# laprade117/interactive-unet

Hardware: AMD Instinct MI355X
Metric: voxels/sec (train step + full-volume predict) on 128^3 chunks (higher is better)
Workload: dtype bf16

## Files before the change

### include/iunet.h

```cpp
#ifndef IUNET_H
#define IUNET_H
#ifdef __cplusplus
extern "C" {
#endif

const char* iunet_last_error(void);
int iunet_abi_version(void);

long long iunet_pack_conv3_elems(int Cout, int Cin, int taps, int mode);
int iunet_pack_conv3(int dtype, const void* w, const void* scale, void* dst, int Cout, int Cin, int taps, int mode,
                     void* stream);
long long iunet_pack_first_conv_elems(int Cout, int Cin, int taps);
int iunet_pack_first_conv(int dtype, const void* w, const void* scale, void* dst, int Cout, int Cin, int taps,
                          void* stream);
int iunet_pack_convT(int dtype, const void* w, void* dst, int Cin, int Cout, int npos, void* stream);

int iunet_pack_desc_bytes(void);
int iunet_pack_batch(const void* descs, int n, int quant_max_cout, void* stream);

int iunet_conv3_fwd(int dtype, int nd, const void* x, long long x_sstride, void* y, long long y_sstride,
                    const void* wpk, const void* bias, void* stats, int N, int D, int H, int W, int Cin, int Cout,
                    int epi, int layout, void* stream);
int iunet_conv3_pick_layout(int nd, int N, int D, int H, int W, int Cin, int Cout);
int iunet_conv3_tile_pairs(int nd, int N, int D, int H, int W, int Cin, int Cout);
// ... 235 lines not shown
int iunet_conv3_dgrad_sample_bnstats(int dtype, int nd, const void* dy, long long dy_sstride, void* dz, long long dz_sstride, const void* wpk,
                                     void* stats, const void* yp, long long yp_sstride, const void* mean, const void* invstd, const void* scale,
                                     const void* shift, int N, int D, int H, int W, int Cin, int Cout, int layout, void* stream);
int iunet_gn_relu_bwd_rows(int dtype, const void* dz, long long dz_ss, const void* y, long long y_ss, void* dy, long long dy_ss,
                           const void* gamma, int groups, const void* scale, const void* shift, const void* mean, const void* invstd,
                           void* dgamma, void* dbeta, void* slab, int rows, void* coef, int C, int N, long long vox, void* stream);
int iunet_gn_relu_pool_bwd(int dtype, int nd, const void* dskip, long long ds_ss, const void* dpool, long long dp_ss, const void* y,
                           long long y_ss, void* dy, long long dy_ss, const void* gamma, int groups, const void* scale, const void* shift,
                           const void* mean, const void* invstd, void* dgamma, void* dbeta, void* slab, void* coef, int C, int N, int Do,
                           int Ho, int Wo, void* stream);
int iunet_bn_relu_pool_bwd(int dtype, int nd, const void* dskip, long long ds_ss, const void* dpool, long long dp_ss,
                           const void* y, long long y_ss, void* dy, long long dy_ss, const void* mean, const void* invstd,
                           const void* gamma, const void* scale, const void* shift, void* dgamma, void* dbeta, void* slab,
                           void* coef, int C, int N, int Do, int Ho, int Wo, void* stream);
int iunet_maxpool_bwd(int dtype, int nd, const void* z, long long z_ss, const void* dpool, long long dp_ss, void* dz,
                      long long dz_ss, int add_skip, int C, int N, int Do, int Ho, int Wo, void* stream);
int iunet_head_loss_num_parts(int N, long long vox);
int iunet_head_loss_fwd(int dtype, const void* x, long long x_ss, int C0, const void* w, const void* bias, int ncls,
                        const void* target, const void* weight, int tdtype, int kind, void* slab, void* out4, void* coef,
                        int N, long long vox, void* stream);
int iunet_head_loss_bwd_num_parts(int N, long long vox, int ncls, int C0);
int iunet_head_loss_bwd(int dtype, const void* x, long long x_ss, int C0, const void* w, const void* bias, int ncls,
                        const void* target, const void* weight, int tdtype, const void* coef, float loss_scale, void* dx,
                        long long dx_ss, void* dwslab, int N, long long vox, void* stream);
int iunet_head_loss_fwd_act(int dtype, const void* x, long long x_ss, int C0, const void* w, const void* bias, int ncls,
                            const void* target, const void* weight, int tdtype, int kind, void* slab, void* out4, void* coef,
                            const void* in_scale, const void* in_shift, int N, long long vox, void* stream);
int iunet_head_loss_bwd_act(int dtype, const void* x, long long x_ss, int C0, const void* w, const void* bias, int ncls,
                            const void* target, const void* weight, int tdtype, const void* coef, float loss_scale, void* dx,
                            long long dx_ss, void* dwslab, const void* in_scale, const void* in_shift, int N, long long vox,
                            void* stream);
int iunet_reduce_slab(void* slab, int nparts, long long n, void* out, float alpha, int accumulate, void* stream);
int iunet_conv3_wgrad_blocks(int nd, int N, int D, int H, int W, int Cin, int Cout);
long long iunet_conv3_wgrad_slab_floats(int nd, int N, int D, int H, int W, int Cin, int Cout);
int iunet_conv3_wgrad(int dtype, int nd, const void* x, long long x_ss, const void* dy, long long dy_ss, void* slab,
                      void* dW, float alpha, int N, int D, int H, int W, int Cin, int Cout, void* stream);
int iunet_conv3_wgrad_act(int dtype, int nd, const void* x, long long x_ss, const void* dy, long long dy_ss, void* slab,
                          void* dW, float alpha, const void* x_scale, const void* x_shift, int N, int D, int H, int W,
                          int Cin, int Cout, void* stream);
int iunet_pack_convT_dgrad(int dtype, const void* w, void* dst, int Cin, int Cout, int npos, void* stream);
int iunet_convT_dgrad(int dtype, int nd, const void* dy, long long dy_ss, void* dx, long long dx_ss, const void* wpk,
                      int N, int D, int H, int W, int Cin, int Cout, void* stream);
int iunet_convT_wgrad_blocks(int nd, int N, int D, int H, int W, int Cin, int Cout);
int iunet_convT_wgrad(int dtype, int nd, const void* x, long long x_ss, const void* dy, long long dy_ss, void* wslab,
                      void* bslab, void* dW, void* db, int N, int D, int H, int W, int Cin, int Cout, void* stream);
int iunet_first_conv_wgrad_blocks(int nd, int N, int D, int H, int W);
int iunet_first_conv_wgrad(int dtype, int nd, const void* x, int in_dtype, const long long* in_strides, const void* dy,
                           long long dy_ss, void* slab, void* dW, int N, int D, int H, int W, int Cin, int Cout,
                           void* stream);
int iunet_first_conv_wgrad_bn(int dtype, int nd, const void* x, int in_dtype, const long long* in_strides, const void* dz,
                              long long dz_ss, const void* y, long long y_ss, const void* mean, const void* invstd,
                              const void* coef, const void* scale, const void* shift, void* slab, void* dW, int N, int D, int H,
                              int W, int Cin, int Cout, void* stream);
int iunet_check_finite(const void* g, long long n, void* flag, void* stream);
int iunet_adamw_step(void* p, const void* g, void* m, void* v, long long n, float lr, float b1, float b2, float eps,
                     float wd, int step, float grad_scale_inv, const void* skip_flag, void* stream);

int iunet_train_state_init(void* state, float loss_scale, int dynamic, void* stream);
int iunet_head_loss_bwd_dev(int dtype, const void* x, long long x_ss, int C0, const void* w, const void* bias, int ncls,
                            const void* target, const void* weight, int tdtype, const void* coef, const void* state, void* dx,
                            long long dx_ss, void* dwslab, const void* in_scale, const void* in_shift, int N, long long vox,
                            void* stream);
int iunet_head_bn_bwd_ok(int C0, int ncls);
int iunet_head_bn_bwd(int dtype, const void* y, long long y_ss, int C0, const void* w, const void* bias, int ncls, const void* target,
                      const void* weight, int tdtype, const void* coef, float loss_scale, const void* state, const void* scale,
                      const void* shift, const void* mean, const void* invstd, const void* gamma, void* dgamma, void* dbeta, void* dy,
                      long long dy_ss, void* dwslab, void* bnslab, void* bncoef, void* dl_scratch, int N, long long vox, void* stream);
int iunet_head_gn_bwd(int dtype, const void* y, long long y_ss, int C0, const void* w, const void* bias, int ncls, const void* target,
                      const void* weight, int tdtype, const void* coef, float loss_scale, const void* state, const void* scale,
                      const void* shift, const void* mean, const void* invstd, const void* gamma, int groups, void* dgamma, void* dbeta, void* dy,
                      long long dy_ss, void* dwslab, void* bnslab, void* bncoef, void* dl_scratch, int N, long long vox, void* stream);
int iunet_head_loss_fwd_act_ps(int dtype, const void* x, long long x_ss, int C0, const void* w, const void* bias, int ncls,
                               const void* target, const void* weight, int tdtype, int kind, void* slab, void* out4, void* coef,
                               const void* in_scale, const void* in_shift, int per_sample, int N, long long vox, void* stream);
int iunet_head_grad_scatter(const void* row, void* dw, void* db, int ncls, int C0, void* stream);
int iunet_adamw_step_dev(void* p, const void* g, void* m, void* v, long long n, float lr, float b1, float b2, float eps, float wd,
                         void* state, int check, float world, void* stream);

typedef struct iunet_train iunet_train;
int iunet_train_create(int dim, int levels, int base, int cin, int ncls, int dtype, int loss_kind, iunet_train** out);
int iunet_train_create_ex(int dim, int levels, int base, int cin, int ncls, int dtype, int loss_kind, int norm, int groups, iunet_train** out);
int iunet_train_create_nested(int dim, int levels, int base, int cin, int ncls, int dtype, int loss_kind, iunet_train** out);
void iunet_train_destroy(iunet_train* t);
long long iunet_train_num_params(const iunet_train* t);
int iunet_train_num_tensors(const iunet_train* t);
int iunet_train_param(const iunet_train* t, int index, char* name, int name_cap, long long* offset, long long* numel);
int iunet_train_num_bn(const iunet_train* t);
long long iunet_train_packed_bytes(const iunet_train* t);
long long iunet_train_workspace_bytes(const iunet_train* t, int N, int D, int H, int W);
int iunet_train_bind(iunet_train* t, void* flat, void* grad, void* m, void* v, void* const* running, void* packed, void* state, void* stream);
int iunet_train_repack(iunet_train* t, void* stream);
int iunet_train_forward_backward(iunet_train* t, const void* x, int in_dtype, const long long* in_strides, const void* target,
                                 const void* weight, int tdtype, int N, int D, int H, int W, void* workspace, void* out4, void* stream);
typedef void (*iunet_train_hook)(void* ctx, int stage);
int iunet_train_forward_backward_hooks(iunet_train* t, const void* x, int in_dtype, const long long* in_strides, const void* target,
                                       const void* weight, int tdtype, int N, int D, int H, int W, void* workspace, void* out4,
                                       iunet_train_hook hook, void* hook_ctx, void* stream);
int iunet_train_update(iunet_train* t, float lr, float b1, float b2, float eps, float wd, float world, void* stream);
int iunet_train_step(iunet_train* t, const void* x, int in_dtype, const long long* in_strides, const void* target, const void* weight,
                     int tdtype, int N, int D, int H, int W, void* workspace, float lr, float b1, float b2, float eps, float wd, void* out4,
                     void* stream);

long long iunet_lk_pack_elems(int nd, int kind, int Cout, int Cin);
int iunet_lk_pack(int dtype, int nd, int kind, const void* w, const void* gamma, const void* beta, const void* mean, const void* var,
                  float eps, void* dst, void* bias_out, int Cout, int Cin, void* stream);
int iunet_lk_stats_parts(int nd, int kind, int N, int D, int H, int W, int Cout);
// ... 100 lines not shown
```

### interactive-unet_amd/csrc/train_misc.hip

```cpp
#include "common.h"

namespace {


struct ConvTDgradParams {
  const void* dy; long long dy_ss;
  void* dx; long long dx_ss;
  const void* wpk;
  int N, D, H, W, Cin, Cout;
};

template <typename T, int ND>
__global__ __launch_bounds__(256) void convT_dgrad_kernel(ConvTDgradParams p) {
  using V8 = V8T<T>;
  constexpr int NPOS = ND == 3 ? 8 : 4;
  const int lane = threadIdx.x & 63, wave = threadIdx.x >> 6;
  const int l15 = lane & 15, q = lane >> 4;
  const int xg = (p.W + 15) / 16;
  const long long rows = (long long)p.D * p.H * xg;
  const long long wid = (long long)blockIdx.x * 4 + wave;
  if (wid >= rows * p.N) return;
  const int n = (int)(wid / rows);
  const long long r = wid - n * rows;
  const int xb = (int)(r % xg), y = (int)((r / xg) % p.H), z = (int)(r / ((long long)xg * p.H));
// ... 280 lines not shown
      for (int t = 0; t < 2; ++t)
#pragma unroll
        for (int u = 0; u < 2; ++u)
#pragma unroll
          for (int j = 0; j < 4; ++j) ws[s * 1024 + (t * 16 + 4 * g + j) * 32 + u * 16 + i16] = acc[c][i][t][u][j];
    }
  }
  if (blockIdx.y == 0) {
    __syncthreads();
    float* red = (float*)smem;
#pragma unroll
    for (int j = 0; j < 8; ++j) red[tid * 8 + j] = bacc[j];
    __syncthreads();
    if (tid < 32) {
      const int pl = tid >> 3, j = tid & 7;
      float sum = 0.f;
      for (int k = pl; k < 256; k += 4) sum += red[k * 8 + j];
      p.bslab[(long long)blockIdx.x * p.Cout + cob * 32 + pl * 8 + j] = sum;
    }
  }
}

__global__ __launch_bounds__(256) void convT_wgrad_reduce_kernel(const float* __restrict__ slab, int nb, int Cin, int Cout, int npos,
                                                                 float* __restrict__ dW) {
  __shared__ f32x4 red[16][16];
  const long long per_b4 = (long long)Cin * Cout * npos / 4;
  const int col4 = threadIdx.x & 15, grp = threadIdx.x >> 4;
  const long long j4 = (long long)blockIdx.x * 16 + col4;
  const f32x4* slab4 = (const f32x4*)slab;
  f32x4 s = f32x4{0.f, 0.f, 0.f, 0.f};
  for (int b = grp; b < nb; b += 16) s += slab4[b * per_b4 + j4];
  red[grp][col4] = s;
  __syncthreads();
  if (grp != 0) return;
#pragma unroll
  for (int g = 1; g < 16; ++g) s += red[g][col4];
  const int ncob = Cout / 32;
#pragma unroll
  for (int k = 0; k < 4; ++k) {
    const long long j = j4 * 4 + k;
    const int c = (int)(j & 31), r = (int)((j >> 5) & 31);
    long long t = j >> 10;
    const int pos = (int)(t % npos); t /= npos;
    const int cob = (int)(t % ncob), cib = (int)(t / ncob);
    dW[((long long)(cib * 32 + r) * Cout + cob * 32 + c) * npos + pos] = s[k];
  }
}

struct FirstWgradParams {
  const void* x; long long sN, sC, sD, sH, sW; int in_dtype;
  const void* dy; long long dy_ss;
  const void* yraw; long long y_ss;
  const float* mean; const float* invstd; const float* coef; const float* scale; const float* shift;
  float* slab;
  int N, D, H, W, Cin, Cout;
  int tilesZ, tilesY, tilesX;
};

__device__ __forceinline__ float load_in2(const void* p, long long off, int dt) {
  switch (dt) {
    case 0: return ((const float*)p)[off];
    case 1: return (float)((const f16*)p)[off];
    case 2: return (float)((const unsigned char*)p)[off] / 255.0f;
    default: return (float)((const bf16*)p)[off];
  }
}

template <typename T, int ND, int CIN>
__global__ __launch_bounds__(256, 2) void first_wgrad_kernel(FirstWgradParams p) {
  using V8 = V8T<T>;
  constexpr int TZ = ND == 3 ? 4 : 1, TY = ND == 3 ? 8 : 16, TX = ND == 3 ? 16 : 32, PADZ = ND == 3 ? 1 : 0;
  constexpr int PZ = TZ + 2 * PADZ, PY = TY + 2, PX = TX + 2, NPIX = PZ * PY * PX, NVOX = TZ * TY * TX;
  constexpr int TAPS = ND == 3 ? 27 : 9, KK = TAPS * CIN, NT = (KK + 15) / 16, KKP = NT * 16;
  constexpr int FX = TX / 16, NKS = NVOX / 32;
  constexpr int PLANE_Y = NVOX * 16 + 64;
  constexpr int XS_BYTES = ((CIN * NPIX * 2 + 255) / 256) * 256;
  extern __shared__ __attribute__((aligned(256))) unsigned char smem[];
  T* xs = (T*)smem;
  unsigned char* dys = smem + XS_BYTES;
  __shared__ __attribute__((aligned(16))) float par[7 * 32];
  if (p.yraw != nullptr && threadIdx.x < 7 * 32) {
    const int k = threadIdx.x >> 5, c = blockIdx.y * 32 + (threadIdx.x & 31);
    par[threadIdx.x] = k == 0 ? p.scale[c] : k == 1 ? p.shift[c] : k == 2 ? p.mean[c] : k == 3 ? p.invstd[c] : p.coef[c * 3 + (k - 4)];
  }
  const unsigned lds_y = (unsigned)(size_t)(__attribute__((address_space(3))) unsigned char*)dys;
  const int tid = threadIdx.x, lane = tid & 63;
  const int wave = __builtin_amdgcn_readfirstlane(tid >> 6);
  const int g = lane >> 4, i16 = lane & 15, q = i16 >> 2, pp = i16 & 3, gh = g >> 1, gl = g & 1;
  const int cob = blockIdx.y;
  const unsigned laneY = lds_y + (pp >> 1) * PLANE_Y + (pp & 1) * 8 + (gh * 16 + gl * 8 + q) * 16;
  int col_off[NT];
#pragma unroll
  for (int ct = 0; ct < NT; ++ct) {
    const int kk = ct * 16 + i16, kc = kk < KK ? kk : 0;
    const int tap = kc / CIN, c = kc % CIN;
    const int dz = ND == 3 ? tap / 9 : 0, dy_ = (tap / 3) % 3, dx = tap % 3;
    col_off[ct] = c * NPIX + (dz * PY + dy_) * PX + dx;
  }
  f32x4 acc[2][NT];
#pragma unroll
  for (int t = 0; t < 2; ++t)
#pragma unroll
    for (int ct = 0; ct < NT; ++ct) acc[t][ct] = f32x4{0, 0, 0, 0};
  const int tps = p.tilesZ * p.tilesY * p.tilesX, ntiles = tps * p.N;
  const long long plane = (long long)p.D * p.H * p.W * 8;
  constexpr int XIT = (NPIX * CIN + 255) / 256, YIT = NVOX * 4 / 256;
  float xr[XIT];
  u32x4 yr[YIT], yw[YIT];
  unsigned oky = 0;
  auto load_tile = [&](int tile) {
    oky = 0;
    const int n = tile / tps;
    int trem = tile - n * tps;
    const int tz_i = trem / (p.tilesY * p.tilesX);
    trem -= tz_i * p.tilesY * p.tilesX;
    const int ty_i = trem / p.tilesX, tx_i = trem - ty_i * p.tilesX;
    const int z0 = tz_i * TZ, y0 = ty_i * TY, x0 = tx_i * TX;
#pragma unroll
    for (int k = 0; k < XIT; ++k) {
      const int it = tid + k * 256;
      const int c = it / NPIX, pix = it - c * NPIX;
      const int px = pix % PX, t2 = pix / PX, py = t2 % PY, pz = t2 / PY;
      const int gz = z0 + pz - PADZ, gy = y0 + py - 1, gx = x0 + px - 1;
      float v = 0.f;
      if (it < NPIX * CIN && (unsigned)gz < (unsigned)p.D && (unsigned)gy < (unsigned)p.H && (unsigned)gx < (unsigned)p.W)
        v = load_in2(p.x, n * p.sN + c * p.sC + gz * p.sD + gy * p.sH + gx * p.sW, p.in_dtype);
      xr[k] = v;
    }
    const T* dyin = (const T*)p.dy + (long long)n * p.dy_ss + (long long)cob * 4 * plane;
#pragma unroll
    for (int it = 0; it < YIT; ++it) {
      const int idx = tid + it * 256, pl = idx / NVOX, pix = idx - pl * NVOX;
      const int px = pix % TX, t2 = pix / TX, py = t2 % TY, pz = t2 / TY;
      const int gz = z0 + pz, gy = y0 + py, gx = x0 + px;
      u32x4 v = u32x4{0u, 0u, 0u, 0u};
      if (gz < p.D && gy < p.H && gx < p.W) v = *(const u32x4*)(dyin + pl * plane + (((long long)gz * p.H + gy) * p.W + gx) * 8);
      yr[it] = v;
      oky |= (gz < p.D && gy < p.H && gx < p.W) ? (1u << it) : 0u;
      if (p.yraw != nullptr) {
        u32x4 w = u32x4{0u, 0u, 0u, 0u};
        if (gz < p.D && gy < p.H && gx < p.W)
          w = *(const u32x4*)((const T*)p.yraw + (long long)n * p.y_ss + (long long)(cob * 4 + pl) * plane + (((long long)gz * p.H + gy) * p.W + gx) * 8);
        yw[it] = w;
      }
    }
  };
  auto commit_tile = [&]() {
#pragma unroll
    for (int k = 0; k < XIT; ++k) {
      const int it = tid + k * 256;
      if (it < NPIX * CIN) xs[it] = from_f32<T>(xr[k]);
    }
#pragma unroll
    for (int it = 0; it < YIT; ++it) {
      const int idx = tid + it * 256, pl = idx / NVOX, pix = idx - pl * NVOX;
      u32x4 v = yr[it];
      if (p.yraw != nullptr && ((oky >> it) & 1u)) {
        const V8 g = __builtin_bit_cast(V8, v), yy = __builtin_bit_cast(V8, yw[it]);
        V8 o;
        const f32x4* pp = (const f32x4*)(par + pl * 8);
        float cs[7][8];
#pragma unroll
        for (int k = 0; k < 7; ++k) {
          const f32x4 lo = pp[k * 8], hi = pp[k * 8 + 1];
#pragma unroll
          for (int j = 0; j < 4; ++j) { cs[k][j] = lo[j]; cs[k][4 + j] = hi[j]; }
        }
#pragma unroll
        for (int j = 0; j < 8; ++j) {
          const float yv = to_f32<T>(yy[j]);
          const float zv = to_f32<T>(from_f32<T>(fmaf(cs[0][j], yv, cs[1][j])));
          const float d = zv > 0.f ? to_f32<T>(g[j]) : 0.f;
          const float xh = (yv - cs[2][j]) * cs[3][j];
          o[j] = from_f32<T>(cs[4][j] * (d - cs[5][j] - xh * cs[6][j]));
        }
        v = __builtin_bit_cast(u32x4, o);
      }
      *(u32x4*)(dys + pl * PLANE_Y + pix * 16) = v;
    }
  };
  if ((int)blockIdx.x < ntiles) load_tile(blockIdx.x);
  for (int tile = blockIdx.x; tile < ntiles; tile += gridDim.x) {
    __syncthreads();
    commit_tile();
    __syncthreads();
    if (tile + (int)gridDim.x < ntiles) load_tile(tile + gridDim.x);
    for (int ks = wave; ks < NKS; ks += 4) {
      const int f = 2 * ks + gh;
      const int xh = f % FX, row = f / FX, fy = row % TY, fz = row / TY;
      const int vbase = (fz * PY + fy) * PX + xh * 16 + gl * 8;
      const V8 a0 = tr_frag2<T>(laneY + (unsigned)(2 * ks * 256), 64);
      const V8 a1 = tr_frag2<T>(laneY + (unsigned)(2 * ks * 256) + 2 * PLANE_Y, 64);
#pragma unroll
      for (int ct = 0; ct < NT; ++ct) {
        V8 b;
#pragma unroll
        for (int j = 0; j < 8; ++j) b[j] = xs[vbase + j + col_off[ct]];
        acc[0][ct] = mfma16<T>(a0, b, acc[0][ct]);
        acc[1][ct] = mfma16<T>(a1, b, acc[1][ct]);
      }
    }
  }
  __syncthreads();
  float* red = (float*)smem;
#pragma unroll
  for (int t = 0; t < 2; ++t)
#pragma unroll
    for (int ct = 0; ct < NT; ++ct)
#pragma unroll
      for (int j = 0; j < 4; ++j) red[(wave * 32 + t * 16 + 4 * g + j) * KKP + ct * 16 + i16] = acc[t][ct][j];
  __syncthreads();
  float* slab = p.slab + ((long long)blockIdx.x * p.Cout + cob * 32) * KKP;
  for (int i = tid; i < 32 * KKP; i += 256)
    slab[i] = red[i] + red[32 * KKP + i] + red[2 * 32 * KKP + i] + red[3 * 32 * KKP + i];
}

__global__ __launch_bounds__(256) void first_wgrad_reduce_kernel(const float* __restrict__ slab, int nb, int Cout, int Cin, int taps,
                                                                 int KKP, float* __restrict__ dW) {
  __shared__ float red[8][32];
  const int total = Cout * Cin * taps;
  const int o = threadIdx.x & 31, grp = threadIdx.x >> 5;
  const int i = blockIdx.x * 32 + o;
  float s = 0.f;
  if (i < total) {
    const int tap = i % taps, c = (i / taps) % Cin, co = i / (taps * Cin);
// ... 78 lines not shown

int iunet_convT_wgrad_blocks(int nd, int N, int D, int H, int W, int Cin, int Cout) {
  if (N < 1 || D < 1 || H < 1 || W < 1 || Cin < 32 || Cout < 32) return 0;
  const int TZ = nd == 3 ? 2 : 1, TY = nd == 3 ? 4 : 8, TX = 16;
  const long long ntiles = (long long)N * ((D + TZ - 1) / TZ) * ((H + TY - 1) / TY) * ((W + TX - 1) / TX);
  const int nci = (Cin / 32) % 2 == 0 ? 2 : 1;
  const int pairs = (Cin / 32 / nci) * (Cout / 32);
  long long nb = (512 + pairs - 1) / pairs;
  if (nb > ntiles) nb = ntiles;
  return (int)(nb < 1 ? 1 : nb);
}

int iunet_convT_wgrad(int dtype, int nd, const void* x, long long x_ss, const void* dy, long long dy_ss, void* wslab,
                      void* bslab, void* dW, void* db, int N, int D, int H, int W, int Cin, int Cout, void* stream) {
  DT_OK(dtype);
  IUNET_REQUIRE(x && dy && wslab && bslab && dW && db, "convT_wgrad: null pointer");
  IUNET_REQUIRE(Cin >= 32 && Cout >= 32 && Cin % 32 == 0 && Cout % 32 == 0, "convT_wgrad: channels must be positive multiples of 32");
  IUNET_REQUIRE(nd == 2 || nd == 3, "convT_wgrad: nd must be 2 or 3");
  IUNET_REQUIRE_GRID("convT_wgrad", N, D, H, W);
  ConvTWgradParams p;
  p.x = x; p.x_ss = x_ss; p.dy = dy; p.dy_ss = dy_ss; p.wslab = (float*)wslab; p.bslab = (float*)bslab;
  p.N = N; p.D = D; p.H = H; p.W = W; p.Cin = Cin; p.Cout = Cout;
  const int TZ = nd == 3 ? 2 : 1, TY = nd == 3 ? 4 : 8, TX = 16;
  p.tilesZ = (D + TZ - 1) / TZ; p.tilesY = (H + TY - 1) / TY; p.tilesX = (W + TX - 1) / TX;
  const int nb = iunet_convT_wgrad_blocks(nd, N, D, H, W, Cin, Cout);
  const int npos = nd == 3 ? 8 : 4;
  const int nvi = 128, nvo = nd == 3 ? 1024 : 512;
  const int lds = 4 * (nvi * 16 + 64) + 4 * (nvo * 16 + 64);
  const int nci = (Cin / 32) % 2 == 0 ? 2 : 1;
  dim3 grid(nb, Cin / 32 / nci, Cout / 32);
#define CTW(TT, NDV) do { if (nci == 2) { IUNET_SET_MAX_LDS((convT_wgrad_kernel<TT, NDV, 2>), lds); \
      hipLaunchKernelGGL((convT_wgrad_kernel<TT, NDV, 2>), grid, dim3(256), lds, (hipStream_t)stream, p); } \
    else { IUNET_SET_MAX_LDS((convT_wgrad_kernel<TT, NDV, 1>), lds); \
      hipLaunchKernelGGL((convT_wgrad_kernel<TT, NDV, 1>), grid, dim3(256), lds, (hipStream_t)stream, p); } } while (0)
  if (dtype == 0) { if (nd == 3) CTW(f16, 3); else CTW(f16, 2); } else { if (nd == 3) CTW(bf16, 3); else CTW(bf16, 2); }
#undef CTW
  const long long total = (long long)Cin * Cout * npos;
  hipLaunchKernelGGL(convT_wgrad_reduce_kernel, dim3((unsigned)(total / 64)), dim3(256), 0, (hipStream_t)stream,
                     (const float*)wslab, nb, Cin, Cout, npos, (float*)dW);
  IUNET_CHECK_HIP(hipGetLastError());
  return iunet_reduce_slab(bslab, nb, Cout, db, 1.0f, 0, stream);
}

int iunet_first_conv_wgrad_blocks(int nd, int N, int D, int H, int W) {
  if (N < 1 || D < 1 || H < 1 || W < 1) return 0;
  const int TZ = nd == 3 ? 4 : 1, TY = nd == 3 ? 8 : 16, TX = nd == 3 ? 16 : 32;
  const long long ntiles = (long long)N * ((D + TZ - 1) / TZ) * ((H + TY - 1) / TY) * ((W + TX - 1) / TX);
  return (int)(ntiles < 512 ? ntiles : 512);
}

static int first_wgrad_impl(int dtype, int nd, const void* x, int in_dtype, const long long* in_strides, const void* dy,
                            long long dy_ss, void* slab, void* dW, int N, int D, int H, int W, int Cin, int Cout,
                            const void* yraw, long long y_ss, const float* mean, const float* invstd, const float* coef,
                            const float* scale, const float* shift, void* stream) {
  DT_OK(dtype);
  IUNET_REQUIRE(x && dy && slab && dW && in_strides, "first_conv_wgrad: null pointer");
  IUNET_REQUIRE(Cin >= 1 && Cin <= 4 && Cout >= 32 && Cout % 32 == 0, "first_conv_wgrad: Cin 1..4, Cout a positive multiple of 32");
  IUNET_REQUIRE(nd == 2 || nd == 3, "first_conv_wgrad: nd must be 2 or 3");
  IUNET_REQUIRE(in_dtype >= 0 && in_dtype <= 3, "first_conv_wgrad: bad input dtype %d", in_dtype);
  IUNET_REQUIRE_GRID("first_conv_wgrad", N, D, H, W);
  FirstWgradParams p;
  p.x = x; p.sN = in_strides[0]; p.sC = in_strides[1]; p.sD = in_strides[2]; p.sH = in_strides[3]; p.sW = in_strides[4];
  p.in_dtype = in_dtype; p.dy = dy; p.dy_ss = dy_ss; p.slab = (float*)slab;
  p.yraw = yraw; p.y_ss = y_ss; p.mean = mean; p.invstd = invstd; p.coef = coef; p.scale = scale; p.shift = shift;
  p.N = N; p.D = D; p.H = H; p.W = W; p.Cin = Cin; p.Cout = Cout;
  const int TZ = nd == 3 ? 4 : 1, TY = nd == 3 ? 8 : 16, TX = nd == 3 ? 16 : 32;
  p.tilesZ = (D + TZ - 1) / TZ; p.tilesY = (H + TY - 1) / TY; p.tilesX = (W + TX - 1) / TX;
  const int nb = iunet_first_conv_wgrad_blocks(nd, N, D, H, W);
  const int taps = nd == 3 ? 27 : 9, KKP = ((taps * Cin + 15) / 16) * 16;
  const int npix = (nd == 3 ? 6 : 1) * (TY + 2) * (TX + 2);
  const int xs_bytes = ((Cin * npix * 2 + 255) / 256) * 256;
  int lds = xs_bytes + 4 * (512 * 16 + 64);
  if (lds < 4 * 32 * KKP * 4) lds = 4 * 32 * KKP * 4;
  dim3 grid(nb, Cout / 32);
#define FW(TT, NDV, CI) do { IUNET_SET_MAX_LDS((first_wgrad_kernel<TT, NDV, CI>), lds); \
    hipLaunchKernelGGL((first_wgrad_kernel<TT, NDV, CI>), grid, dim3(256), lds, (hipStream_t)stream, p); } while (0)
#define FW_CIN(TT, NDV) switch (Cin) { case 1: FW(TT, NDV, 1); break; case 2: FW(TT, NDV, 2); break; case 3: FW(TT, NDV, 3); break; default: FW(TT, NDV, 4); break; }
  if (dtype == 0) { if (nd == 3) { FW_CIN(f16, 3) } else { FW_CIN(f16, 2) } }
  else            { if (nd == 3) { FW_CIN(bf16, 3) } else { FW_CIN(bf16, 2) } }
#undef FW_CIN
#undef FW
  const int total = Cout * Cin * taps;
  hipLaunchKernelGGL(first_wgrad_reduce_kernel, dim3((total + 31) / 32), dim3(256), 0, (hipStream_t)stream,
                     (const float*)slab, nb, Cout, Cin, taps, KKP, (float*)dW);
  IUNET_CHECK_HIP(hipGetLastError());
  return IUNET_OK;
}

int iunet_first_conv_wgrad(int dtype, int nd, const void* x, int in_dtype, const long long* in_strides, const void* dy,
                           long long dy_ss, void* slab, void* dW, int N, int D, int H, int W, int Cin, int Cout,
                           void* stream) {
  return first_wgrad_impl(dtype, nd, x, in_dtype, in_strides, dy, dy_ss, slab, dW, N, D, H, W, Cin, Cout, nullptr, 0, nullptr,
                          nullptr, nullptr, nullptr, nullptr, stream);
}

int iunet_first_conv_wgrad_bn(int dtype, int nd, const void* x, int in_dtype, const long long* in_strides, const void* dz,
                              long long dz_ss, const void* y, long long y_ss, const void* mean, const void* invstd,
                              const void* coef, const void* scale, const void* shift, void* slab, void* dW, int N, int D, int H,
                              int W, int Cin, int Cout, void* stream) {
  IUNET_REQUIRE(y && mean && invstd && coef && scale && shift, "first_conv_wgrad_bn: null pointer");
  return first_wgrad_impl(dtype, nd, x, in_dtype, in_strides, dz, dz_ss, slab, dW, N, D, H, W, Cin, Cout, y, y_ss,
                          (const float*)mean, (const float*)invstd, (const float*)coef, (const float*)scale,
                          (const float*)shift, stream);
}

}
```

### interactive-unet_amd/csrc/train_net.hip

```cpp
#include "common.h"
#include "pack_desc.h"
#include <algorithm>
#include <cstdio>
#include <cstdlib>
#include <string>
#include <vector>

namespace {

long long align256(long long v) { return (v + 255) & ~255ll; }
bool env_on(const char* name) { const char* e = getenv(name); return e != nullptr && e[0] != 0; }

struct TParam { std::string name; long long off, numel; };

struct TPack {
  int cout = 0, cin = 0, dg = 0;
  long long buf[2] = {-1, -1};
  long long elems[2] = {0, 0};
};

struct TConv {
  std::string name;
  int ci, co, l, first;
  long long w, gamma, beta;
// ... 545 lines not shown
                             WS + L.dy, (long long)c0 * v0, F(L.hslab), F(L.bnslab), F(L.bncoef), WS + L.dz[kl] ,
                             N, v0, stream);
      dy_ready = kl;
    } else if (n->head_act)
      rc = iunet_head_loss_bwd_dev(dt, WS + L.y[kl], (long long)c0 * v0, c0, P + n->head_w, P + n->head_b, n->ncls, target, weight, tdtype, F(L.coef),
                                   n->state, WS + L.dz[kl], (long long)c0 * v0, F(L.hslab), F(L.scale[kl]), F(L.shift[kl]), N, v0, stream);
    else
      rc = iunet_head_loss_bwd_dev(dt, WS + L.z[kl], (long long)c0 * v0, c0, P + n->head_w, P + n->head_b, n->ncls, target, weight, tdtype, F(L.coef),
                                   n->state, WS + L.dz[kl], (long long)c0 * v0, F(L.hslab), nullptr, nullptr, N, v0, stream);
    if (rc) return rc;
    rc = iunet_reduce_slab(F(L.hslab), nparts, (long long)n->ncls * (c0 + 1), F(L.htmp), 1.0f, 0, stream);
    if (rc) return rc;
    rc = iunet_head_grad_scatter(F(L.htmp), G + n->head_w, G + n->head_b, n->ncls, c0, stream);
    if (rc) return rc;
  }
  auto conv_bwd = [&](int k, const void* dzp, long long dz_ss, const void* xp, long long x_ss, void* dxp, long long dx_ss, int x_act,
                      const void* dpool, long long dpool_ss, int feeds) -> int {
    const TConv& c = n->conv[k];
    int d, h, w;
    dims(c.l, d, h, w);
    const long long v = vox(c.l);
    void* dy = WS + L.dy;
    const void* y = WS + L.y[k];
    if (k == dy_ready) {
    } else if (n->norm == 1 && dpool != nullptr) {
      int dn, hn, wn;
      dims(c.l + 1, dn, hn, wn);
      rc = iunet_gn_relu_pool_bwd(dt, dim, dzp, dz_ss, dpool, dpool_ss, y, c.co * v, dy, c.co * v, P + c.gamma, n->groups, F(L.scale[k]), F(L.shift[k]),
                                  F(L.mean[k]), F(L.invstd[k]), G + c.gamma, G + c.beta, F(L.bnslab), F(L.bncoef), c.co, N, dn, hn, wn, stream);
    } else if (n->norm == 1) {
      const int rows = bw_ready[k] > 0 ? bw_ready[k] : 0;
      bw_ready[k] = -1;
      rc = iunet_gn_relu_bwd_rows(dt, dzp, dz_ss, y, c.co * v, dy, c.co * v, P + c.gamma, n->groups, F(L.scale[k]), F(L.shift[k]), F(L.mean[k]), F(L.invstd[k]),
                                  G + c.gamma, G + c.beta, rows > 0 ? F(L.stats) : F(L.bnslab), rows, F(L.bncoef), c.co, N, v, stream);
    } else if (dpool != nullptr) {
      int dn, hn, wn;
      dims(c.l + 1, dn, hn, wn);
      rc = iunet_bn_relu_pool_bwd(dt, dim, dzp, dz_ss, dpool, dpool_ss, y, c.co * v, dy, c.co * v, F(L.mean[k]), F(L.invstd[k]), P + c.gamma,
                                  F(L.scale[k]), F(L.shift[k]), G + c.gamma, G + c.beta, F(L.bnslab), F(L.bncoef), c.co, N, dn, hn, wn, stream);
    } else if (bw_ready[k] >= 0) {
      const int nparts = bw_ready[k];
      bw_ready[k] = -1;
      rc = iunet_bn_relu_bwd_apply(dt, dzp, dz_ss, y, c.co * v, c.first ? nullptr : dy, c.co * v, F(L.mean[k]), F(L.invstd[k]), P + c.gamma,
                                   F(L.scale[k]), F(L.shift[k]), G + c.gamma, G + c.beta, F(L.stats), nparts, F(L.bncoef), c.co, N, v, stream);
    } else {
      rc = iunet_bn_relu_bwd(dt, dzp, dz_ss, nullptr, dz_ss, y, c.co * v, c.first ? nullptr : dy, c.co * v, F(L.mean[k]), F(L.invstd[k]), P + c.gamma,
                             F(L.scale[k]), F(L.shift[k]), G + c.gamma, G + c.beta, F(L.bnslab), F(L.bncoef), c.co, N, v, stream);
    }
    if (rc) return rc;
    float* gw = G + c.w;
    if (c.first && n->norm == 1)
      return iunet_first_conv_wgrad(dt, dim, x, in_dtype, in_strides, dy, c.co * v, F(L.wslab), gw, N, d, h, w, c.ci, c.co, stream);
    if (c.first)
      return iunet_first_conv_wgrad_bn(dt, dim, x, in_dtype, in_strides, dzp, dz_ss, y, c.co * v, F(L.mean[k]), F(L.invstd[k]), F(L.bncoef),
                                       F(L.scale[k]), F(L.shift[k]), F(L.wslab), gw, N, d, h, w, c.ci, c.co, stream);
    if (x_act < 0) rc = iunet_conv3_wgrad(dt, dim, xp, x_ss, dy, c.co * v, F(L.wslab), gw, 1.0f, N, d, h, w, c.ci, c.co, stream);
    else rc = iunet_conv3_wgrad_act(dt, dim, xp, x_ss, dy, c.co * v, F(L.wslab), gw, 1.0f, F(L.scale[x_act]), F(L.shift[x_act]), N, d, h, w, c.ci,
                                    c.co, stream);
    if (rc) return rc;
    long long woff;
    int fused = 0;
    const int lay = pack_pick(c.dgr, dim, N, d, h, w, false, feeds >= 0 && (n->fuse_bw || n->gn_bw), &woff, &fused);
    if (lay < 0) return lay;
    if (fused && n->fuse_bw) {
      rc = iunet_conv3_dgrad_bnstats_lay(dt, dim, dy, c.co * v, dxp, dx_ss, K + woff, F(L.stats), WS + L.y[feeds], c.ci * v, F(L.mean[feeds]),
                                         F(L.invstd[feeds]), F(L.scale[feeds]), F(L.shift[feeds]), N, d, h, w, c.co, c.ci, lay, stream);
      bw_ready[feeds] = iunet_conv3_stats_parts(dim, N, d, h, w, c.ci, 2);
    } else {
      int gn_rows = 0;
      if (n->norm == 1 && fused && n->gn_bw)
        gn_rows = iunet_conv3_sample_stats_rows(dt, dim, N, d, h, w, c.co, c.ci, lay);
      if (gn_rows > 0) {
        rc = iunet_conv3_dgrad_sample_bnstats(dt, dim, dy, c.co * v, dxp, dx_ss, K + woff, F(L.stats), WS + L.y[feeds], c.ci * v, F(L.mean[feeds]),
                                              F(L.invstd[feeds]), F(L.scale[feeds]), F(L.shift[feeds]), N, d, h, w, c.co, c.ci, lay, stream);
        bw_ready[feeds] = gn_rows;
      } else {
        rc = iunet_conv3_fwd(dt, dim, dy, c.co * v, dxp, dx_ss, K + woff, nullptr, nullptr, N, d, h, w, c.co, c.ci, 0, lay, stream);
      }
    }
    return rc;
  };
  if (n->nested) {
    auto node_conv2_bwd = [&](int s, int i, int m, const void* dpool, long long dpool_ss) -> int {
      const long long v = vox(i);
      const int c = n->ch[i], k1 = 2 * s, k2 = k1 + 1;
      const bool fused = conv2_fused(i);
      const void* x2 = fused ? (const void*)(WS + L.y[k1]) : (const void*)(WS + L.z[k1]);
      const void* dzp = nullptr;
      long long dz_ss = 0;
      if (k2 != dy_ready) {
        const void* sp[8];
        long long ss[8];
        int K_ = 0;
        for (int jj = m + 1; jj < lv - i; ++jj) {
          const int q = n->node_at[i * lv + jj];
          sp[K_] = WS + L.ndcat[q] + (long long)m * c * v * 2; ss[K_++] = (long long)(jj + 1) * c * v;
        }
        if (i >= 1) { sp[K_] = WS + L.dT[n->node_at[(i - 1) * lv + m + 1]]; ss[K_++] = (long long)c * v; }
        if (K_ + (dpool != nullptr) == 1) {
          dzp = sp[0]; dz_ss = ss[0];
        } else {
          const TConv& cc = n->conv[k2];
          int d, h, w;
          dims(i, d, h, w);
          rc = iunet_bn_relu_sum_bwd(dt, dim, K_, sp, ss, dpool, dpool_ss, WS + L.y[k2], (long long)c * v, WS + L.dy, (long long)c * v, F(L.mean[k2]),
                                     F(L.invstd[k2]), P + cc.gamma, F(L.scale[k2]), F(L.shift[k2]), G + cc.gamma, G + cc.beta, F(L.bnslab), F(L.bncoef),
                                     c, N, d, h, w, stream);
          if (rc) return rc;
// ... 111 lines not shown
```

### interactive-unet_amd/interactive_unet/train_engine.py

```python
import ctypes
import math

import os

import torch

from . import _native as nv
from . import topology
from .engine import BN_EPS
from .topology import _vox, check_spatial

LOSS_KINDS = {'ce': 0, 'dice': 1, 'iou': 2, 'mcc': 3, 'dice_ce': 4, 'iou_ce': 5, 'mcc_ce': 6}
BN_MOMENTUM = 0.1


def metrics(out4, sync):
    if not sync:
        return out4
    o = out4.tolist()
    return {'Loss': o[0], 'Dice': o[1], 'IoU': o[2], 'MCC': o[3]}


class TrainEngineBase:

# ... 375 lines not shown
                    nv.ptr(ws['out4']), nv.ptr(ws['coef']), nv.ptr(ws['scale.' + act]), nv.ptr(ws['shift.' + act]),
                    int(self.gn), N, vox, nv.stream())
        return tdt, w

    def _stage_conv_bwd(self, ws, name, dz_ptr, dz_ss, z_ptr, z_ss, x_ptr, x_ss, ci, co, l, dx_ptr, dx_ss, N,
                        x_raw=None, x_act=None, pool_bwd=None, feeds=None, dy_ready=False):
        d = ws['dims'][l]
        v = _vox(d)
        s = nv.stream()
        bn = name.replace('conv', 'bn')
        dy = ws['dy']
        first = name == 'enc0.conv1'
        if dy_ready:
            pass
        elif self.gn and pool_bwd is not None:
            dp_ptr, dp_ss, do = pool_bwd
            nv.call('iunet_gn_relu_pool_bwd', self.dt, self.dim, dz_ptr, dz_ss, dp_ptr, dp_ss, self._P(ws['y.' + name]), co * v, self._P(dy), co * v,
                    nv.ptr(self.p(bn + '.weight')), self.groups, nv.ptr(ws['scale.' + name]), nv.ptr(ws['shift.' + name]),
                    nv.ptr(ws['mean.' + name]), nv.ptr(ws['invstd.' + name]), nv.ptr(self.g(bn + '.weight')),
                    nv.ptr(self.g(bn + '.bias')), nv.ptr(ws['bnslab']), nv.ptr(ws['bncoef']), co, N, do[0], do[1], do[2], s)
        elif self.gn:
            rows = self._bw_ready.pop(name, 0)
            nv.call('iunet_gn_relu_bwd_rows', self.dt, dz_ptr, dz_ss, self._P(ws['y.' + name]), co * v, self._P(dy), co * v,
                    nv.ptr(self.p(bn + '.weight')), self.groups, nv.ptr(ws['scale.' + name]), nv.ptr(ws['shift.' + name]),
                    nv.ptr(ws['mean.' + name]), nv.ptr(ws['invstd.' + name]), nv.ptr(self.g(bn + '.weight')),
                    nv.ptr(self.g(bn + '.bias')), nv.ptr(ws['stats'] if rows > 0 else ws['bnslab']), rows, nv.ptr(ws['bncoef']), co, N, v, s)
        elif pool_bwd is not None:
            dp_ptr, dp_ss, do = pool_bwd
            nv.call('iunet_bn_relu_pool_bwd', self.dt, self.dim, dz_ptr, dz_ss, dp_ptr, dp_ss, self._P(ws['y.' + name]), co * v,
                    self._P(dy), co * v, nv.ptr(ws['mean.' + name]), nv.ptr(ws['invstd.' + name]),
                    nv.ptr(self.p(bn + '.weight')), nv.ptr(ws['scale.' + name]), nv.ptr(ws['shift.' + name]),
                    nv.ptr(self.g(bn + '.weight')), nv.ptr(self.g(bn + '.bias')),
                    nv.ptr(ws['bnslab']), nv.ptr(ws['bncoef']), co, N, do[0], do[1], do[2], s)
        elif name in self._bw_ready:
            nparts = self._bw_ready.pop(name)
            nv.call('iunet_bn_relu_bwd_apply', self.dt, dz_ptr, dz_ss, self._P(ws['y.' + name]), co * v,
                    None if first else self._P(dy), co * v, nv.ptr(ws['mean.' + name]), nv.ptr(ws['invstd.' + name]),
                    nv.ptr(self.p(bn + '.weight')), nv.ptr(ws['scale.' + name]), nv.ptr(ws['shift.' + name]),
                    nv.ptr(self.g(bn + '.weight')), nv.ptr(self.g(bn + '.bias')), nv.ptr(ws['stats']), nparts,
                    nv.ptr(ws['bncoef']), co, N, v, s)
        else:
            nv.call('iunet_bn_relu_bwd', self.dt, dz_ptr, dz_ss, None, z_ss, self._P(ws['y.' + name]), co * v,
                    None if first else self._P(dy), co * v, nv.ptr(ws['mean.' + name]), nv.ptr(ws['invstd.' + name]),
                    nv.ptr(self.p(bn + '.weight')), nv.ptr(ws['scale.' + name]), nv.ptr(ws['shift.' + name]),
                    nv.ptr(self.g(bn + '.weight')), nv.ptr(self.g(bn + '.bias')),
                    nv.ptr(ws['bnslab']), nv.ptr(ws['bncoef']), co, N, v, s)
        gw = self.g(name + '.weight')
        if first and self.gn:
            x, xs = x_raw
            nv.call('iunet_first_conv_wgrad', self.dt, self.dim, nv.ptr(x), nv.IN_DTYPE_CODE[x.dtype], nv.ll_array(xs),
                    self._P(dy), co * v, nv.ptr(ws['wslab']), nv.ptr(gw), N, d[0], d[1], d[2], ci, co, s)
        elif first:
            x, xs = x_raw
            nv.call('iunet_first_conv_wgrad_bn', self.dt, self.dim, nv.ptr(x), nv.IN_DTYPE_CODE[x.dtype], nv.ll_array(xs),
                    dz_ptr, dz_ss, self._P(ws['y.' + name]), co * v, nv.ptr(ws['mean.' + name]), nv.ptr(ws['invstd.' + name]),
                    nv.ptr(ws['bncoef']), nv.ptr(ws['scale.' + name]), nv.ptr(ws['shift.' + name]),
                    nv.ptr(ws['wslab']), nv.ptr(gw), N, d[0], d[1], d[2], ci, co, s)
        else:
            if x_act is None:
                nv.call('iunet_conv3_wgrad', self.dt, self.dim, x_ptr, x_ss, self._P(dy), co * v, nv.ptr(ws['wslab']),
                        nv.ptr(gw), 1.0, N, d[0], d[1], d[2], ci, co, s)
            else:
                nv.call('iunet_conv3_wgrad_act', self.dt, self.dim, x_ptr, x_ss, self._P(dy), co * v, nv.ptr(ws['wslab']),
                        nv.ptr(gw), 1.0, nv.ptr(ws['scale.' + x_act]), nv.ptr(ws['shift.' + x_act]),
                        N, d[0], d[1], d[2], ci, co, s)
            _, pkd = self.pk[name]
            lay, wd, fused = pkd.pick(self.dim, N, *d, bw=feeds is not None and (self.fuse_bw or self.gn_bw))
            gn_rows = 0
            if self.gn and fused and self.gn_bw:
                gn_rows = nv.lib().iunet_conv3_sample_stats_rows(self.dt, self.dim, N, d[0], d[1], d[2], co, ci, lay)
            if fused and self.fuse_bw:
                nv.call('iunet_conv3_dgrad_bnstats_lay', self.dt, self.dim, self._P(dy), co * v, dx_ptr, dx_ss, nv.ptr(wd),
                        nv.ptr(ws['stats']), self._P(ws['y.' + feeds]), ci * v, nv.ptr(ws['mean.' + feeds]),
                        nv.ptr(ws['invstd.' + feeds]), nv.ptr(ws['scale.' + feeds]), nv.ptr(ws['shift.' + feeds]),
                        N, d[0], d[1], d[2], co, ci, lay, s)
                self._bw_ready[feeds] = nv.lib().iunet_conv3_stats_parts(self.dim, N, d[0], d[1], d[2], ci, 2)
            elif gn_rows > 0:
                nv.call('iunet_conv3_dgrad_sample_bnstats', self.dt, self.dim, self._P(dy), co * v, dx_ptr, dx_ss, nv.ptr(wd),
                        nv.ptr(ws['stats']), self._P(ws['y.' + feeds]), ci * v, nv.ptr(ws['mean.' + feeds]),
                        nv.ptr(ws['invstd.' + feeds]), nv.ptr(ws['scale.' + feeds]), nv.ptr(ws['shift.' + feeds]),
                        N, d[0], d[1], d[2], co, ci, lay, s)
                self._bw_ready[feeds] = gn_rows
            else:
                nv.call('iunet_conv3_fwd', self.dt, self.dim, self._P(dy), co * v, dx_ptr, dx_ss, nv.ptr(wd), None, None,
                        N, d[0], d[1], d[2], co, ci, 0, lay, s)

    def backward(self, ws, x, x_strides, y, w, tdt, N):
        L, ch, dims = self.levels, self.ch, ws['dims']
        s = nv.stream()
        v0 = _vox(dims[0])
        dfeat = ws['dz.dec0.conv2']
        nparts = nv.lib().iunet_head_loss_bwd_num_parts(N, v0, self.ncls, ch[0])
        dy_ready = None
        if self.gn_head:
            bn = 'dec0.bn2'
            nv.call('iunet_head_gn_bwd', self.dt, self._P(ws['y.dec0.conv2']), ch[0] * v0, ch[0], nv.ptr(self.p('head.weight')),
                    nv.ptr(self.p('head.bias')), self.ncls, nv.ptr(y), nv.ptr(w), tdt, nv.ptr(ws['coef']), 0.0, nv.ptr(self.state),
                    nv.ptr(ws['scale.dec0.conv2']), nv.ptr(ws['shift.dec0.conv2']), nv.ptr(ws['mean.dec0.conv2']), nv.ptr(ws['invstd.dec0.conv2']),
                    nv.ptr(self.p(bn + '.weight')), self.groups, nv.ptr(self.g(bn + '.weight')), nv.ptr(self.g(bn + '.bias')), self._P(ws['dy']), ch[0] * v0,
                    nv.ptr(ws['hslab']), nv.ptr(ws['bnslab']), nv.ptr(ws['bncoef']), self._P(dfeat), N, v0, s)
            dy_ready = 'dec0.conv2'
        elif self.head_bn and nv.lib().iunet_head_bn_bwd_ok(ch[0], self.ncls):
            bn = 'dec0.bn2'
            nv.call('iunet_head_bn_bwd', self.dt, self._P(ws['y.dec0.conv2']), ch[0] * v0, ch[0], nv.ptr(self.p('head.weight')),
                    nv.ptr(self.p('head.bias')), self.ncls, nv.ptr(y), nv.ptr(w), tdt, nv.ptr(ws['coef']), 0.0, nv.ptr(self.state),
                    nv.ptr(ws['scale.dec0.conv2']), nv.ptr(ws['shift.dec0.conv2']), nv.ptr(ws['mean.dec0.conv2']), nv.ptr(ws['invstd.dec0.conv2']),
                    nv.ptr(self.p(bn + '.weight')), nv.ptr(self.g(bn + '.weight')), nv.ptr(self.g(bn + '.bias')), self._P(ws['dy']), ch[0] * v0,
                    nv.ptr(ws['hslab']), nv.ptr(ws['bnslab']), nv.ptr(ws['bncoef']), self._P(dfeat), N, v0, s)
# ... 445 lines not shown
```

Baseline: 748.5 million.

## Recompute first conv output in wgrad kernel instead of reading stored activations

The first-layer weight-gradient kernel with BN backward now recomputes the raw first-conv output on the fly with MFMA from the input tile already staged in LDS and the packed forward weights. It no longer reads the stored pre-norm activation tensor. This removes a full-resolution read of the widest activation in exchange for extra matrix work, an added barrier, and more registers for the held weight fragments. It also reassigns how dy tile elements map to threads so they match the MFMA output layout.

```diff
diff --git a/include/iunet.h b/include/iunet.h
--- a/include/iunet.h
+++ b/include/iunet.h
@@ -311,6 +311,10 @@
                               long long dz_ss, const void* y, long long y_ss, const void* mean, const void* invstd,
                               const void* coef, const void* scale, const void* shift, void* slab, void* dW, int N, int D, int H,
                               int W, int Cin, int Cout, void* stream);
+int iunet_first_conv_wgrad_bn_rc(int dtype, int nd, const void* x, int in_dtype, const long long* in_strides, const void* dz,
+                                 long long dz_ss, const void* w, const void* bias, int relu, const void* mean, const void* invstd,
+                                 const void* coef, const void* scale, const void* shift, void* slab, void* dW, int N, int D, int H,
+                                 int W, int Cin, int Cout, void* stream);
 int iunet_check_finite(const void* g, long long n, void* flag, void* stream);
 int iunet_adamw_step(void* p, const void* g, void* m, void* v, long long n, float lr, float b1, float b2, float eps,
                      float wd, int step, float grad_scale_inv, const void* skip_flag, void* stream);
diff --git a/interactive-unet_amd/csrc/train_misc.hip b/interactive-unet_amd/csrc/train_misc.hip
--- a/interactive-unet_amd/csrc/train_misc.hip
+++ b/interactive-unet_amd/csrc/train_misc.hip
@@ -356,6 +356,7 @@
   const void* dy; long long dy_ss;
   const void* yraw; long long y_ss;
   const float* mean; const float* invstd; const float* coef; const float* scale; const float* shift;
+  const void* wfwd; const float* bias;
   float* slab;
   int N, D, H, W, Cin, Cout;
   int tilesZ, tilesY, tilesX;
@@ -370,22 +371,25 @@
   }
 }
 
-template <typename T, int ND, int CIN>
+template <typename T, int ND, int CIN, bool RC>
 __global__ __launch_bounds__(256, 2) void first_wgrad_kernel(FirstWgradParams p) {
   using V8 = V8T<T>;
   constexpr int TZ = ND == 3 ? 4 : 1, TY = ND == 3 ? 8 : 16, TX = ND == 3 ? 16 : 32, PADZ = ND == 3 ? 1 : 0;
   constexpr int PZ = TZ + 2 * PADZ, PY = TY + 2, PX = TX + 2, NPIX = PZ * PY * PX, NVOX = TZ * TY * TX;
   constexpr int TAPS = ND == 3 ? 27 : 9, KK = TAPS * CIN, NT = (KK + 15) / 16, KKP = NT * 16;
   constexpr int FX = TX / 16, NKS = NVOX / 32;
+  constexpr int KS = (KK + 31) / 32;
   constexpr int PLANE_Y = NVOX * 16 + 64;
   constexpr int XS_BYTES = ((CIN * NPIX * 2 + 255) / 256) * 256;
   extern __shared__ __attribute__((aligned(256))) unsigned char smem[];
   T* xs = (T*)smem;
   unsigned char* dys = smem + XS_BYTES;
-  __shared__ __attribute__((aligned(16))) float par[7 * 32];
-  if (p.yraw != nullptr && threadIdx.x < 7 * 32) {
+  __shared__ __attribute__((aligned(16))) float par[8 * 32];
+  const bool bn = RC || p.yraw != nullptr;
+  if (bn) {
     const int k = threadIdx.x >> 5, c = blockIdx.y * 32 + (threadIdx.x & 31);
-    par[threadIdx.x] = k == 0 ? p.scale[c] : k == 1 ? p.shift[c] : k == 2 ? p.mean[c] : k == 3 ? p.invstd[c] : p.coef[c * 3 + (k - 4)];
+    par[threadIdx.x] = k == 0 ? p.scale[c] : k == 1 ? p.shift[c] : k == 2 ? p.mean[c] : k == 3 ? p.invstd[c] : k < 7 ? p.coef[c * 3 + (k - 4)]
+                       : (RC && p.bias != nullptr) ? p.bias[c] : 0.f;
   }
   const unsigned lds_y = (unsigned)(size_t)(__attribute__((address_space(3))) unsigned char*)dys;
   const int tid = threadIdx.x, lane = tid & 63;
@@ -401,6 +405,22 @@
     const int dz = ND == 3 ? tap / 9 : 0, dy_ = (tap / 3) % 3, dx = tap % 3;
     col_off[ct] = c * NPIX + (dz * PY + dy_) * PX + dx;
   }
+  V8 wa[RC ? KS : 1][2];
+  int koff[RC ? KS : 1][8];
+  if constexpr (RC) {
+    const V8* wp = (const V8*)p.wfwd + (long long)cob * KS * 2 * 64 + lane;
+#pragma unroll
+    for (int ks = 0; ks < KS; ++ks) {
+      wa[ks][0] = wp[(ks * 2 + 0) * 64]; wa[ks][1] = wp[(ks * 2 + 1) * 64];
+#pragma unroll
+      for (int j = 0; j < 8; ++j) {
+        const int k = 32 * ks + 8 * g + j, kc = k < KK ? k : 0;
+        const int tap = kc / CIN, c = kc % CIN;
+        const int dz = ND == 3 ? tap / 9 : 0, dy_ = (tap / 3) % 3, dx = tap % 3;
+        koff[ks][j] = c * NPIX + (dz * PY + dy_) * PX + dx;
+      }
+    }
+  }
   f32x4 acc[2][NT];
 #pragma unroll
   for (int t = 0; t < 2; ++t)
@@ -410,7 +430,7 @@
   const long long plane = (long long)p.D * p.H * p.W * 8;
   constexpr int XIT = (NPIX * CIN + 255) / 256, YIT = NVOX * 4 / 256;
   float xr[XIT];
-  u32x4 yr[YIT], yw[YIT];
+  u32x4 yr[YIT], yw[RC ? 1 : YIT];
   unsigned oky = 0;
   auto load_tile = [&](int tile) {
     oky = 0;
@@ -434,14 +454,14 @@
     const T* dyin = (const T*)p.dy + (long long)n * p.dy_ss + (long long)cob * 4 * plane;
 #pragma unroll
     for (int it = 0; it < YIT; ++it) {
-      const int idx = tid + it * 256, pl = idx / NVOX, pix = idx - pl * NVOX;
+      const int pl = g, pix = (wave * YIT + it) * 16 + i16;
       const int px = pix % TX, t2 = pix / TX, py = t2 % TY, pz = t2 / TY;
       const int gz = z0 + pz, gy = y0 + py, gx = x0 + px;
       u32x4 v = u32x4{0u, 0u, 0u, 0u};
       if (gz < p.D && gy < p.H && gx < p.W) v = *(const u32x4*)(dyin + pl * plane + (((long long)gz * p.H + gy) * p.W + gx) * 8);
       yr[it] = v;
       oky |= (gz < p.D && gy < p.H && gx < p.W) ? (1u << it) : 0u;
-      if (p.yraw != nullptr) {
+      if (!RC && p.yraw != nullptr) {
         u32x4 w = u32x4{0u, 0u, 0u, 0u};
         if (gz < p.D && gy < p.H && gx < p.W)
           w = *(const u32x4*)((const T*)p.yraw + (long long)n * p.y_ss + (long long)(cob * 4 + pl) * plane + (((long long)gz * p.H + gy) * p.W + gx) * 8);
@@ -455,12 +475,33 @@
       const int it = tid + k * 256;
       if (it < NPIX * CIN) xs[it] = from_f32<T>(xr[k]);
     }
+    if constexpr (RC) __syncthreads();
 #pragma unroll
     for (int it = 0; it < YIT; ++it) {
-      const int idx = tid + it * 256, pl = idx / NVOX, pix = idx - pl * NVOX;
+      const int pl = g, f = wave * YIT + it, pix = f * 16 + i16;
       u32x4 v = yr[it];
-      if (p.yraw != nullptr && ((oky >> it) & 1u)) {
-        const V8 g = __builtin_bit_cast(V8, v), yy = __builtin_bit_cast(V8, yw[it]);
+      V8 yrc;
+      if constexpr (RC) {
+        const int fx = f % FX, row = f / FX, fy = row % TY, fz = row / TY;
+        const int base = (fz * PY + fy) * PX + fx * 16 + i16;
+        f32x4 c0 = f32x4{0, 0, 0, 0}, c1 = f32x4{0, 0, 0, 0};
+#pragma unroll
+        for (int ks = 0; ks < KS; ++ks) {
+          V8 b;
+#pragma unroll
+          for (int j = 0; j < 8; ++j) b[j] = xs[base + koff[ks][j]];
+          c0 = mfma16<T>(wa[ks][0], b, c0);
+          c1 = mfma16<T>(wa[ks][1], b, c1);
+        }
+        const f32x4* bp = (const f32x4*)(par + 7 * 32 + pl * 8);
+        const f32x4 b0 = bp[0], b1 = bp[1];
+#pragma unroll
+        for (int j = 0; j < 4; ++j) { yrc[j] = from_f32<T>(c0[j] + b0[j]); yrc[4 + j] = from_f32<T>(c1[j] + b1[j]); }
+      }
+      if (bn && ((oky >> it) & 1u)) {
+        V8 yy;
+        if constexpr (RC) yy = yrc; else yy = __builtin_bit_cast(V8, yw[it]);
+        const V8 gv = __builtin_bit_cast(V8, v);
         V8 o;
         const f32x4* pp = (const f32x4*)(par + pl * 8);
         float cs[7][8];
@@ -474,7 +515,7 @@
         for (int j = 0; j < 8; ++j) {
           const float yv = to_f32<T>(yy[j]);
           const float zv = to_f32<T>(from_f32<T>(fmaf(cs[0][j], yv, cs[1][j])));
-          const float d = zv > 0.f ? to_f32<T>(g[j]) : 0.f;
+          const float d = zv > 0.f ? to_f32<T>(gv[j]) : 0.f;
           const float xh = (yv - cs[2][j]) * cs[3][j];
           o[j] = from_f32<T>(cs[4][j] * (d - cs[5][j] - xh * cs[6][j]));
         }
@@ -659,7 +700,7 @@
 static int first_wgrad_impl(int dtype, int nd, const void* x, int in_dtype, const long long* in_strides, const void* dy,
                             long long dy_ss, void* slab, void* dW, int N, int D, int H, int W, int Cin, int Cout,
                             const void* yraw, long long y_ss, const float* mean, const float* invstd, const float* coef,
-                            const float* scale, const float* shift, void* stream) {
+                            const float* scale, const float* shift, const void* wfwd, const float* bias, void* stream) {
   DT_OK(dtype);
   IUNET_REQUIRE(x && dy && slab && dW && in_strides, "first_conv_wgrad: null pointer");
   IUNET_REQUIRE(Cin >= 1 && Cin <= 4 && Cout >= 32 && Cout % 32 == 0, "first_conv_wgrad: Cin 1..4, Cout a positive multiple of 32");
@@ -669,6 +710,7 @@
   FirstWgradParams p;
   p.x = x; p.sN = in_strides[0]; p.sC = in_strides[1]; p.sD = in_strides[2]; p.sH = in_strides[3]; p.sW = in_strides[4];
   p.in_dtype = in_dtype; p.dy = dy; p.dy_ss = dy_ss; p.slab = (float*)slab;
+  p.wfwd = wfwd; p.bias = bias;
   p.yraw = yraw; p.y_ss = y_ss; p.mean = mean; p.invstd = invstd; p.coef = coef; p.scale = scale; p.shift = shift;
   p.N = N; p.D = D; p.H = H; p.W = W; p.Cin = Cin; p.Cout = Cout;
   const int TZ = nd == 3 ? 4 : 1, TY = nd == 3 ? 8 : 16, TX = nd == 3 ? 16 : 32;
@@ -680,13 +722,15 @@
   int lds = xs_bytes + 4 * (512 * 16 + 64);
   if (lds < 4 * 32 * KKP * 4) lds = 4 * 32 * KKP * 4;
   dim3 grid(nb, Cout / 32);
-#define FW(TT, NDV, CI) do { IUNET_SET_MAX_LDS((first_wgrad_kernel<TT, NDV, CI>), lds); \
-    hipLaunchKernelGGL((first_wgrad_kernel<TT, NDV, CI>), grid, dim3(256), lds, (hipStream_t)stream, p); } while (0)
+#define FW_RC(TT, NDV, CI, RCV) do { IUNET_SET_MAX_LDS((first_wgrad_kernel<TT, NDV, CI, RCV>), lds); \
+    hipLaunchKernelGGL((first_wgrad_kernel<TT, NDV, CI, RCV>), grid, dim3(256), lds, (hipStream_t)stream, p); } while (0)
+#define FW(TT, NDV, CI) do { if (wfwd != nullptr) FW_RC(TT, NDV, CI, true); else FW_RC(TT, NDV, CI, false); } while (0)
 #define FW_CIN(TT, NDV) switch (Cin) { case 1: FW(TT, NDV, 1); break; case 2: FW(TT, NDV, 2); break; case 3: FW(TT, NDV, 3); break; default: FW(TT, NDV, 4); break; }
   if (dtype == 0) { if (nd == 3) { FW_CIN(f16, 3) } else { FW_CIN(f16, 2) } }
   else            { if (nd == 3) { FW_CIN(bf16, 3) } else { FW_CIN(bf16, 2) } }
 #undef FW_CIN
 #undef FW
+#undef FW_RC
   const int total = Cout * Cin * taps;
   hipLaunchKernelGGL(first_wgrad_reduce_kernel, dim3((total + 31) / 32), dim3(256), 0, (hipStream_t)stream,
                      (const float*)slab, nb, Cout, Cin, taps, KKP, (float*)dW);
@@ -698,7 +742,7 @@
                            long long dy_ss, void* slab, void* dW, int N, int D, int H, int W, int Cin, int Cout,
                            void* stream) {
   return first_wgrad_impl(dtype, nd, x, in_dtype, in_strides, dy, dy_ss, slab, dW, N, D, H, W, Cin, Cout, nullptr, 0, nullptr,
-                          nullptr, nullptr, nullptr, nullptr, stream);
+                          nullptr, nullptr, nullptr, nullptr, nullptr, nullptr, stream);
 }
 
 int iunet_first_conv_wgrad_bn(int dtype, int nd, const void* x, int in_dtype, const long long* in_strides, const void* dz,
@@ -708,7 +752,21 @@
   IUNET_REQUIRE(y && mean && invstd && coef && scale && shift, "first_conv_wgrad_bn: null pointer");
   return first_wgrad_impl(dtype, nd, x, in_dtype, in_strides, dz, dz_ss, slab, dW, N, D, H, W, Cin, Cout, y, y_ss,
                           (const float*)mean, (const float*)invstd, (const float*)coef, (const float*)scale,
-                          (const float*)shift, stream);
-}
-
-}
+                          (const float*)shift, nullptr, nullptr, stream);
+}
+
+int iunet_first_conv_wgrad_bn_rc(int dtype, int nd, const void* x, int in_dtype, const long long* in_strides, const void* dz,
+                                 long long dz_ss, const void* w, const void* bias, int relu, const void* mean, const void* invstd,
+                                 const void* coef, const void* scale, const void* shift, void* slab, void* dW, int N, int D, int H,
+                                 int W, int Cin, int Cout, void* stream) {
+  IUNET_REQUIRE(w && mean && invstd && coef && scale && shift, "first_conv_wgrad_bn_rc: null pointer");
+  IUNET_REQUIRE(relu == 0, "first_conv_wgrad_bn_rc: the forward's relu form has no raw output to recompute");
+  IUNET_REQUIRE(dtype == 0 || dtype == 1, "first_conv_wgrad_bn_rc: the forward's 16-bit output only (dtype 0 / 1, got %d): its e4m3 form is y rounded once more",
+                dtype);
+  IUNET_REQUIRE(nd == 3 || D == 1, "first_conv_wgrad_bn_rc: 2-D needs D == 1");
+  return first_wgrad_impl(dtype, nd, x, in_dtype, in_strides, dz, dz_ss, slab, dW, N, D, H, W, Cin, Cout, nullptr, 0,
+                          (const float*)mean, (const float*)invstd, (const float*)coef, (const float*)scale,
+                          (const float*)shift, w, (const float*)bias, stream);
+}
+
+}
diff --git a/interactive-unet_amd/csrc/train_net.hip b/interactive-unet_amd/csrc/train_net.hip
--- a/interactive-unet_amd/csrc/train_net.hip
+++ b/interactive-unet_amd/csrc/train_net.hip
@@ -621,8 +621,8 @@
     if (c.first && n->norm == 1)
       return iunet_first_conv_wgrad(dt, dim, x, in_dtype, in_strides, dy, c.co * v, F(L.wslab), gw, N, d, h, w, c.ci, c.co, stream);
     if (c.first)
-      return iunet_first_conv_wgrad_bn(dt, dim, x, in_dtype, in_strides, dzp, dz_ss, y, c.co * v, F(L.mean[k]), F(L.invstd[k]), F(L.bncoef),
-                                       F(L.scale[k]), F(L.shift[k]), F(L.wslab), gw, N, d, h, w, c.ci, c.co, stream);
+      return iunet_first_conv_wgrad_bn_rc(dt, dim, x, in_dtype, in_strides, dzp, dz_ss, K + c.first_pk, nullptr, 0, F(L.mean[k]), F(L.invstd[k]),
+                                          F(L.bncoef), F(L.scale[k]), F(L.shift[k]), F(L.wslab), gw, N, d, h, w, c.ci, c.co, stream);
     if (x_act < 0) rc = iunet_conv3_wgrad(dt, dim, xp, x_ss, dy, c.co * v, F(L.wslab), gw, 1.0f, N, d, h, w, c.ci, c.co, stream);
     else rc = iunet_conv3_wgrad_act(dt, dim, xp, x_ss, dy, c.co * v, F(L.wslab), gw, 1.0f, F(L.scale[x_act]), F(L.shift[x_act]), N, d, h, w, c.ci,
                                     c.co, stream);
diff --git a/interactive-unet_amd/interactive_unet/train_engine.py b/interactive-unet_amd/interactive_unet/train_engine.py
--- a/interactive-unet_amd/interactive_unet/train_engine.py
+++ b/interactive-unet_amd/interactive_unet/train_engine.py
@@ -451,8 +451,8 @@
                     self._P(dy), co * v, nv.ptr(ws['wslab']), nv.ptr(gw), N, d[0], d[1], d[2], ci, co, s)
         elif first:
             x, xs = x_raw
-            nv.call('iunet_first_conv_wgrad_bn', self.dt, self.dim, nv.ptr(x), nv.IN_DTYPE_CODE[x.dtype], nv.ll_array(xs),
-                    dz_ptr, dz_ss, self._P(ws['y.' + name]), co * v, nv.ptr(ws['mean.' + name]), nv.ptr(ws['invstd.' + name]),
+            nv.call('iunet_first_conv_wgrad_bn_rc', self.dt, self.dim, nv.ptr(x), nv.IN_DTYPE_CODE[x.dtype], nv.ll_array(xs),
+                    dz_ptr, dz_ss, nv.ptr(self.pk[name][0]), None, 0, nv.ptr(ws['mean.' + name]), nv.ptr(ws['invstd.' + name]),
                     nv.ptr(ws['bncoef']), nv.ptr(ws['scale.' + name]), nv.ptr(ws['shift.' + name]),
                     nv.ptr(ws['wslab']), nv.ptr(gw), N, d[0], d[1], d[2], ci, co, s)
         else:
```

Result: no change. 750.1 million (median of 6 runs) (+0.2%).
